# jinlinyi/PerspectiveFields

Measured on NVIDIA H100. Metric: images/sec at 640x480 (Paramnet-360Cities-edina), H100 vs ref CPU, higher is better.
Workload: dtype f32 via 3x bf16 split MMA, fp32 accumulate

## Files before the change

perspectivefields_b200/csrc/gemm_tma.cuh:

```cuda
#pragma once
#include <cuda.h>

#include "tc_ptx.cuh"

namespace pf {

constexpr int MODE_GEMM = 0, MODE_HALO = 1;
constexpr int kTmaThreads = 384;
constexpr int kHaloBytes = 180 * 128;

struct TmaGemmParams {
  int M;
  int B, H, W;
  int Cin;
  int N, K;
  int a_c0, a_gc;
  int c_split, a2_c0;
  int groups;
  int b_row0;
  const float* bias; int bias_mode, bias_gstride;
  int act; const float* gamma;
  const float* res;  int ldr, r_coff, r_gcoff, res_relu;
  const float* res2; int ldr2, r2_coff, r2_gcoff;
  float* C; int ldc, c_coff, c_gcoff;
  __nv_bfloat16* Shi; __nv_bfloat16* Slo; int lds, s_coff, s_gcoff, split_relu;
  const float* pred_w; const float* pred_b; float* pred_out; int pred_nc, pred_mode;
  int phase4;
};

template <int BN, int MODE, int KB, bool PP = false, int NP = 3> struct TmaCfg {
  static_assert(KB == 32 || KB == 64, "KB");
  static_assert(BN % 32 == 0 && BN <= 256, "BN");
  static_assert(!PP || MODE == MODE_GEMM, "the ping-pong schedule is a GEMM-mode schedule");
  static_assert(NP == 1 || NP == 3, "NP");
  static constexpr int kPlanes = NP == 3 ? 2 : 1;
  static constexpr int kTileM = PP ? 64 : 128;
  static constexpr int kBPlane = BN * KB * 2;
  static constexpr int kAPlane = kTileM * KB * 2;
  static constexpr int kStage = (MODE == MODE_GEMM ? kPlanes * kAPlane : 0) + kPlanes * kBPlane;
  static constexpr int kABuf = kPlanes * kHtPlaneBytes;
  static constexpr int kAccPitch = 68;
  static constexpr int kAccStage = 2 * 64 * kAccPitch * 4;
  static constexpr int kBudget = 225 * 1024 - kAccStage - (MODE == MODE_HALO ? 2 * kABuf : 0);
  static constexpr int kStagesRaw = kBudget / kStage;
  static constexpr int kStages = kStagesRaw > 16 ? 16 : kStagesRaw;
  static constexpr int kSmemBytes = (MODE == MODE_HALO ? 2 * kABuf : 0) + kStages * kStage + kAccStage + 512 + 1024;
  static_assert(kStages >= 2, "ring too shallow");
  static_assert(kSmemBytes <= 227 * 1024, "shared memory per block");
};

__device__ __forceinline__ void mbar_expect_tx(uint32_t bar, uint32_t bytes) {
  asm volatile("mbarrier.arrive.expect_tx.shared::cta.b64 _, [%0], %1;\n" ::"r"(bar), "r"(bytes) : "memory");
}
__device__ __forceinline__ void tma_load_2d(uint32_t dst, const CUtensorMap* map, uint32_t bar, int c0, int c1) {
  asm volatile("cp.async.bulk.tensor.2d.shared::cluster.global.mbarrier::complete_tx::bytes [%0], [%1, {%3, %4}], [%2];\n"
               ::"r"(dst), "l"(reinterpret_cast<uint64_t>(map)), "r"(bar), "r"(c0), "r"(c1) : "memory");
}
__device__ __forceinline__ void tma_load_4d(uint32_t dst, const CUtensorMap* map, uint32_t bar, int c0, int c1, int c2, int c3) {
  asm volatile("cp.async.bulk.tensor.4d.shared::cluster.global.mbarrier::complete_tx::bytes [%0], [%1, {%3, %4, %5, %6}], [%2];\n"
               ::"r"(dst), "l"(reinterpret_cast<uint64_t>(map)), "r"(bar), "r"(c0), "r"(c1), "r"(c2), "r"(c3) : "memory");
}
__device__ __forceinline__ void tma_prefetch_desc(const CUtensorMap* map) {
  asm volatile("prefetch.tensormap [%0];\n" ::"l"(reinterpret_cast<uint64_t>(map)) : "memory");
}

struct TmaMaps {
  CUtensorMap a_hi, a_lo, a2_hi, a2_lo, b_hi, b_lo;
};

template <int BN, int MODE, int KB, bool PP = false, int NP = 3>
__global__ void __launch_bounds__(kTmaThreads, 1) gemm_tma_kernel(const __grid_constant__ TmaMaps maps, const TmaGemmParams p, int tiles_x, int tiles_y) {
  using Cfg = TmaCfg<BN, MODE, KB, PP, NP>;
  constexpr bool kLo = NP == 3;
  constexpr int NS = Cfg::kStages;
  constexpr int SPC = 9 * (64 / KB);
  constexpr int kConsumerWarps = PP ? 4 : 8;
  extern __shared__ unsigned char smem_dyn[];
  const uint32_t raw = smem_u32(smem_dyn);
  const uint32_t sbase = (raw + 1023u) & ~1023u;
  unsigned char* sm = smem_dyn + (sbase - raw);
  const uint32_t a_base = sbase;
  const uint32_t ring = sbase + (MODE == MODE_HALO ? 2 * Cfg::kABuf : 0);
  const uint32_t acc_base = ring + NS * Cfg::kStage;
  const uint32_t bars = acc_base + Cfg::kAccStage;
  auto full_b = [&](int s) { return bars + 8u * s; };
  auto empty_b = [&](int s) { return bars + 8u * (NS + s); };
  auto full_a = [&](int i) { return bars + 8u * (2 * NS + i); };
  auto empty_a = [&](int i) { return bars + 8u * (2 * NS + 2 + i); };
  auto order_b = [&](int w) { return bars + 8u * (2 * NS + 4 + w); };

  const int tid = threadIdx.x, lane = tid & 31, warp = tid >> 5;
  const int n_tiles = cdiv(p.N, BN);
  const int m_tiles = MODE == MODE_GEMM ? cdiv(p.M, Cfg::kTileM) : p.B * tiles_x * tiles_y;
  const int total_tiles = m_tiles * n_tiles * p.groups;
  const int nchunks = MODE == MODE_HALO ? p.Cin / 64 : 0;
  const int nk = MODE == MODE_GEMM ? p.K / KB : nchunks * SPC;
  const bool b_resident = MODE == MODE_HALO && nchunks == 1 && SPC <= NS;

  if (tid == 0) {
    tma_prefetch_desc(&maps.a_hi); tma_prefetch_desc(&maps.b_hi);
    if (kLo) { tma_prefetch_desc(&maps.a_lo); tma_prefetch_desc(&maps.b_lo); }
    for (int s = 0; s < NS; ++s) { mbar_init(full_b(s), 1); mbar_init(empty_b(s), kConsumerWarps); }
    for (int i = 0; i < 2; ++i) { mbar_init(full_a(i), 1); mbar_init(empty_a(i), kConsumerWarps); mbar_init(order_b(i), 4); }
    fence_mbar_init();
  }
  __syncthreads();
  pdl_wait();
  pdl_launch();

  auto decode = [&](int tile, int& mt, int& g, int& n0) {
    n0 = (tile % n_tiles) * BN;
    tile /= n_tiles;
    g = tile % p.groups;
    mt = tile / p.groups;
  };

  if (warp < 4) {
    asm volatile("setmaxnreg.dec.sync.aligned.u32 40;\n");
    if (warp == 0 && lane == 0) {
      int it = 0;
      for (int tile = blockIdx.x; tile < total_tiles; tile += gridDim.x) {
        int mt, g, n0;
        decode(tile, mt, g, n0);
        const int brow = p.b_row0 + g * p.N + n0;
        if (b_resident && it > 0) break;
        for (int kc = 0; kc < nk; ++kc, ++it) {
          const int s = it % NS;
          mbar_wait(empty_b(s), ((it / NS) & 1) ^ 1);
          mbar_expect_tx(full_b(s), Cfg::kStage);
          const uint32_t st = ring + s * Cfg::kStage;
          int kcol;
          if (MODE == MODE_GEMM) {
            kcol = kc * KB;
            tma_load_2d(st, &maps.a_hi, full_b(s), p.a_c0 + g * p.a_gc + kcol, mt * Cfg::kTileM);
            if (kLo) tma_load_2d(st + Cfg::kAPlane, &maps.a_lo, full_b(s), p.a_c0 + g * p.a_gc + kcol, mt * Cfg::kTileM);
          } else {
            const int c = kc / SPC, u = kc - c * SPC;
            kcol = KB == 32 ? (u >> 1) * p.Cin + c * 64 + (u & 1) * 32 : u * p.Cin + c * 64;
          }
          const uint32_t bdst = st + (MODE == MODE_GEMM ? Cfg::kPlanes * Cfg::kAPlane : 0);
          tma_load_2d(bdst, &maps.b_hi, full_b(s), kcol, brow);
          if (kLo) tma_load_2d(bdst + Cfg::kBPlane, &maps.b_lo, full_b(s), kcol, brow);
        }
      }
    } else if (MODE == MODE_HALO && warp == 1 && lane == 0) {
      int ita = 0;
      for (int tile = blockIdx.x; tile < total_tiles; tile += gridDim.x) {
        int mt, g, n0;
        decode(tile, mt, g, n0);
        const int tx = mt % tiles_x, ty = (mt / tiles_x) % tiles_y, bimg = mt / (tiles_x * tiles_y);
        for (int c = 0; c < nchunks; ++c, ++ita) {
          const int buf = ita & 1;
          mbar_wait(empty_a(buf), ((ita >> 1) & 1) ^ 1);
          mbar_expect_tx(full_a(buf), Cfg::kPlanes * kHaloBytes);
          const uint32_t dst = a_base + buf * Cfg::kABuf;
          const int ci = c * 64;
          if (p.c_split > 0 && ci >= p.c_split) {
            tma_load_4d(dst, &maps.a2_hi, full_a(buf), p.a2_c0 + ci - p.c_split, tx * kHtTileW - 1, ty * kHtTileH - 1, bimg);
            if (kLo) tma_load_4d(dst + kHtPlaneBytes, &maps.a2_lo, full_a(buf), p.a2_c0 + ci - p.c_split, tx * kHtTileW - 1, ty * kHtTileH - 1, bimg);
          } else {
            tma_load_4d(dst, &maps.a_hi, full_a(buf), p.a_c0 + g * p.a_gc + ci, tx * kHtTileW - 1, ty * kHtTileH - 1, bimg);
            if (kLo) tma_load_4d(dst + kHtPlaneBytes, &maps.a_lo, full_a(buf), p.a_c0 + g * p.a_gc + ci, tx * kHtTileW - 1, ty * kHtTileH - 1, bimg);
          }
        }
      }
    }
    return;
  }

  asm volatile("setmaxnreg.inc.sync.aligned.u32 232;\n");
  const int wg = (warp >> 2) - 1;
  const int wt = tid & 127;
  float* stage = reinterpret_cast<float*>(sm + (acc_base - sbase)) + wg * 64 * Cfg::kAccPitch;
  const int erow = wt & 63, eh = wt >> 6;
  const int r = PP ? erow : wg * 64 + erow;
  constexpr int kTileStep = PP ? 2 : 1;
  float acc[BN / 2];
  int it = 0, ita = 0;
  for (int tl = PP ? wg : 0, tile = blockIdx.x + tl * gridDim.x; tile < total_tiles; tile += kTileStep * gridDim.x, tl += kTileStep) {
    int mt, g, n0;
    decode(tile, mt, g, n0);
    if (PP) {
      it = tl * nk;
      if (tl > 0) mbar_wait(order_b(wg ^ 1), ((tl - 1) >> 1) & 1);
    }
    int prev_s = -1, prev_buf = -1;
    fence_regs(acc);
    for (int kc = 0; kc < nk; ++kc, ++it) {
      const int s = it % NS;
      uint32_t a_hi, a_lo;
      bool chunk_end = false;
      int buf = 0;
      if (MODE == MODE_HALO) {
        const int c = kc / SPC, u = kc - c * SPC;
        const int tap = KB == 32 ? (u >> 1) : u, ky = tap / 3, kx = tap - ky * 3;
        buf = ita & 1;
        if (u == 0) mbar_wait(full_a(buf), (ita >> 1) & 1);
        a_hi = a_base + buf * Cfg::kABuf + ((ky + 8 * wg) * kHtHaloW + kx) * 128 + (KB == 32 ? (u & 1) * 64 : 0);
        a_lo = a_hi + kHtPlaneBytes;
        chunk_end = u == SPC - 1;
      } else {
        a_hi = ring + s * Cfg::kStage + (PP ? 0 : wg * 64 * KB * 2);
        a_lo = a_hi + Cfg::kAPlane;
      }
      const int sb = b_resident ? kc : s;
      if (!b_resident || tl == 0) mbar_wait(full_b(sb), b_resident ? 0 : ((it / NS) & 1));
      const uint32_t b_hi = ring + sb * Cfg::kStage + (MODE == MODE_GEMM ? Cfg::kPlanes * Cfg::kAPlane : 0);
      const uint64_t dah = MODE == MODE_HALO ? ht_a_desc(a_hi) : wgmma_tile_desc<KB>(a_hi);
      const uint64_t dbh = wgmma_tile_desc<KB>(b_hi);
      wgmma_fence();
      if (kLo) {
        const uint64_t dal = MODE == MODE_HALO ? ht_a_desc(a_lo) : wgmma_tile_desc<KB>(a_lo);
        const uint64_t dbl = wgmma_tile_desc<KB>(b_hi + Cfg::kBPlane);
#pragma unroll
        for (int kk = 0; kk < KB / 16; ++kk) {
          const uint32_t first = (kc | kk) ? 1u : 0u;
          wgmma_bf16<BN>(acc, dal + 2 * kk, dbh + 2 * kk, first);
          wgmma_bf16<BN>(acc, dah + 2 * kk, dbl + 2 * kk, 1u);
          wgmma_bf16<BN>(acc, dah + 2 * kk, dbh + 2 * kk, 1u);
        }
      } else {
#pragma unroll
        for (int kk = 0; kk < KB / 16; ++kk) wgmma_bf16<BN>(acc, dah + 2 * kk, dbh + 2 * kk, (kc | kk) ? 1u : 0u);
      }
      wgmma_commit();
      wgmma_wait<1>();
      if (lane == 0 && prev_s >= 0) {
        if (!b_resident) mbar_arrive(empty_b(prev_s));
        if (MODE == MODE_HALO && prev_buf >= 0) mbar_arrive(empty_a(prev_buf));
      }
      prev_s = s;
      prev_buf = chunk_end ? buf : -1;
      if (MODE == MODE_HALO && chunk_end) ++ita;
    }
    if (PP && lane == 0) mbar_arrive(order_b(wg));
    wgmma_wait<0>();
    fence_regs(acc);
    if (lane == 0 && prev_s >= 0) {
      if (!b_resident) mbar_arrive(empty_b(prev_s));
      if (MODE == MODE_HALO && prev_buf >= 0) mbar_arrive(empty_a(prev_buf));
    }

    long long m;
    bool valid;
    int cls_off = 0;
    int bimg = 0, oy = 0, ox = 0;
    if (MODE == MODE_GEMM) {
      m = (long long)mt * Cfg::kTileM + r;
      valid = m < p.M;
    } else {
      const int tx = mt % tiles_x, ty = (mt / tiles_x) % tiles_y;
      bimg = mt / (tiles_x * tiles_y);
      oy = ty * kHtTileH + (r >> 3); ox = tx * kHtTileW + (r & 7);
      valid = oy < p.H && ox < p.W;
      m = ((long long)bimg * p.H + oy) * p.W + ox;
      if (p.bias_mode == 2) {
        const int ry = oy == 0 ? 0 : (oy == p.H - 1 ? 2 : 1);
        const int rx = ox == 0 ? 0 : (ox == p.W - 1 ? 2 : 1);
        cls_off = (ry * 3 + rx) * p.N;
      }
    }
    const float* __restrict__ bias = p.bias ? p.bias + (long long)g * p.bias_gstride : nullptr;
    const int frow = (wt >> 5) * 16 + (lane >> 2), fcol = 2 * (lane & 3);
#pragma unroll
    for (int rd = 0; rd < (BN + 63) / 64; ++rd) {
      named_bar_sync(1 + wg, 128);
#pragma unroll
      for (int jb = 0; jb < 8; ++jb) {
        const int cb = rd * 8 + jb;
        if (cb < BN / 8) {
          float* d0 = stage + frow * Cfg::kAccPitch + jb * 8 + fcol;
          *reinterpret_cast<float2*>(d0) = make_float2(acc[4 * cb], acc[4 * cb + 1]);
          *reinterpret_cast<float2*>(d0 + 8 * Cfg::kAccPitch) = make_float2(acc[4 * cb + 2], acc[4 * cb + 3]);
        }
      }
      named_bar_sync(1 + wg, 128);
      const int ch = 2 * rd + eh;
      const bool ph4 = MODE == MODE_HALO && BN == 128 && p.phase4;
      const bool staged_split = p.Shi && !ph4;
      float o[32];
      if (ch < BN / 32) {
        const int nb = n0 + ch * 32;
        const long long mo = ph4 ? ((long long)bimg * 2 * p.H + 2 * oy + (ch >> 1)) * (2 * p.W) + 2 * ox + (ch & 1) : m;
        const int nbo = ph4 ? 0 : nb;
        const bool chunk_ok = nb < p.N;
        const float* srow = stage + erow * Cfg::kAccPitch + eh * 32;
#pragma unroll
        for (int j = 0; j < 32; j += 4) {
          const float4 t = *reinterpret_cast<const float4*>(srow + j);
          o[j] = t.x; o[j + 1] = t.y; o[j + 2] = t.z; o[j + 3] = t.w;
        }
        if (valid && chunk_ok) {
          if (p.bias_mode) {
#pragma unroll
            for (int j = 0; j < 32; j += 4) {
              const float4 bv = __ldg(reinterpret_cast<const float4*>(bias + cls_off + nb + j));
              o[j] += bv.x; o[j + 1] += bv.y; o[j + 2] += bv.z; o[j + 3] += bv.w;
            }
          }
          if (p.act == 1) {
#pragma unroll
            for (int j = 0; j < 32; ++j) o[j] = fmaxf(o[j], 0.f);
          } else if (p.act == 2) {
#pragma unroll
            for (int j = 0; j < 32; ++j) o[j] = gelu_erf(o[j]);
          }
          if (p.gamma) {
#pragma unroll
            for (int j = 0; j < 32; j += 4) {
              const float4 gv = __ldg(reinterpret_cast<const float4*>(p.gamma + nb + j));
              o[j] *= gv.x; o[j + 1] *= gv.y; o[j + 2] *= gv.z; o[j + 3] *= gv.w;
            }
          }
          if (p.res) {
            const float* rp = p.res + m * p.ldr + p.r_coff + g * p.r_gcoff + nb;
#pragma unroll
            for (int j = 0; j < 32; j += 4) {
              float4 rv = *reinterpret_cast<const float4*>(rp + j);
              if (p.res_relu) { rv.x = fmaxf(rv.x, 0.f); rv.y = fmaxf(rv.y, 0.f); rv.z = fmaxf(rv.z, 0.f); rv.w = fmaxf(rv.w, 0.f); }
              o[j] += rv.x; o[j + 1] += rv.y; o[j + 2] += rv.z; o[j + 3] += rv.w;
            }
          }
          if (p.res2) {
            const float* rp = p.res2 + m * p.ldr2 + p.r2_coff + g * p.r2_gcoff + nb;
#pragma unroll
            for (int j = 0; j < 32; j += 4) {
              const float4 rv = *reinterpret_cast<const float4*>(rp + j);
              o[j] += rv.x; o[j + 1] += rv.y; o[j + 2] += rv.z; o[j + 3] += rv.w;
            }
          }
          if (MODE == MODE_HALO && (BN == 32 || BN == 128) && p.pred_w) {
            float v0 = __ldg(p.pred_b), v1 = p.pred_nc > 1 ? __ldg(p.pred_b + 1) : 0.f;
#pragma unroll
            for (int j = 0; j < 32; j += 4) {
              const float4 w0 = __ldg(reinterpret_cast<const float4*>(p.pred_w + j));
              v0 = fmaf(o[j], w0.x, v0); v0 = fmaf(o[j + 1], w0.y, v0); v0 = fmaf(o[j + 2], w0.z, v0); v0 = fmaf(o[j + 3], w0.w, v0);
              if (p.pred_nc > 1) {
                const float4 w1 = __ldg(reinterpret_cast<const float4*>(p.pred_w + 32 + j));
                v1 = fmaf(o[j], w1.x, v1); v1 = fmaf(o[j + 1], w1.y, v1); v1 = fmaf(o[j + 2], w1.z, v1); v1 = fmaf(o[j + 3], w1.w, v1);
              }
            }
            const long long HWl = (long long)p.H * p.W * (ph4 ? 4 : 1);
            const long long bi = mo / HWl, pix = mo - bi * HWl;
            float* po = p.pred_out + bi * p.pred_nc * HWl + pix;
            if (p.pred_mode == 1) {
              const float nrm = fmaxf(sqrtf(v0 * v0 + v1 * v1), 1e-12f);
              po[0] = v0 / nrm; po[HWl] = v1 / nrm;
            } else {
              po[0] = fminf(fmaxf(v0, -1.f), 1.f);
            }
          }
        }
        if (chunk_ok && (p.C || (p.Shi && !staged_split))) {
          const bool odd = lane & 1;
          const bool valid_p = __shfl_xor_sync(0xffffffffu, (int)valid, 1) != 0;
          const long long mo_p = mo + (odd ? -1 : 1) * (ph4 ? 2 : 1);
          const long long moA = odd ? mo_p : mo, moB = odd ? mo : mo_p;
          const bool vA = odd ? valid_p : valid, vB = odd ? valid : valid_p;
          if (p.C) {
            float* cA = p.C + moA * p.ldc + p.c_coff + g * p.c_gcoff + nbo + (odd ? 4 : 0);
            float* cB = p.C + moB * p.ldc + p.c_coff + g * p.c_gcoff + nbo + (odd ? 4 : 0);
#pragma unroll
            for (int t = 0; t < 4; ++t) {
              float k[4], rr[4];
#pragma unroll
              for (int e = 0; e < 4; ++e) {
                k[e] = odd ? o[8 * t + 4 + e] : o[8 * t + e];
                rr[e] = __shfl_xor_sync(0xffffffffu, odd ? o[8 * t + e] : o[8 * t + 4 + e], 1);
              }
              if (vA) *reinterpret_cast<float4*>(cA + 8 * t) = odd ? make_float4(rr[0], rr[1], rr[2], rr[3]) : make_float4(k[0], k[1], k[2], k[3]);
              if (vB) *reinterpret_cast<float4*>(cB + 8 * t) = odd ? make_float4(k[0], k[1], k[2], k[3]) : make_float4(rr[0], rr[1], rr[2], rr[3]);
            }
          }
          if (p.Shi && !staged_split) {
            const long long sA = moA * p.lds + p.s_coff + g * p.s_gcoff + nbo + (odd ? 8 : 0);
            const long long sB = moB * p.lds + p.s_coff + g * p.s_gcoff + nbo + (odd ? 8 : 0);
#pragma unroll
            for (int t = 0; t < 2; ++t) {
              float k[8], rr[8];
#pragma unroll
              for (int e = 0; e < 8; ++e) {
                const float mine = odd ? o[16 * t + 8 + e] : o[16 * t + e], give = odd ? o[16 * t + e] : o[16 * t + 8 + e];
                k[e] = p.split_relu ? fmaxf(mine, 0.f) : mine;
                rr[e] = __shfl_xor_sync(0xffffffffu, p.split_relu ? fmaxf(give, 0.f) : give, 1);
              }
              uint4 kh, kl, rh, rl;
              split_bf16x2(k[0], k[1], kh.x, kl.x); split_bf16x2(k[2], k[3], kh.y, kl.y);
              split_bf16x2(k[4], k[5], kh.z, kl.z); split_bf16x2(k[6], k[7], kh.w, kl.w);
              split_bf16x2(rr[0], rr[1], rh.x, rl.x); split_bf16x2(rr[2], rr[3], rh.y, rl.y);
              split_bf16x2(rr[4], rr[5], rh.z, rl.z); split_bf16x2(rr[6], rr[7], rh.w, rl.w);
              if (vA) {
                *reinterpret_cast<uint4*>(p.Shi + sA + 16 * t) = odd ? rh : kh;
                *reinterpret_cast<uint4*>(p.Slo + sA + 16 * t) = odd ? rl : kl;
              }
              if (vB) {
                *reinterpret_cast<uint4*>(p.Shi + sB + 16 * t) = odd ? kh : rh;
                *reinterpret_cast<uint4*>(p.Slo + sB + 16 * t) = odd ? kl : rl;
              }
            }
          }
        }
      }
      if (staged_split) {
        named_bar_sync(1 + wg, 128);
        unsigned char* sS = reinterpret_cast<unsigned char*>(stage);
        if (ch < BN / 32) {
#pragma unroll
          for (int t = 0; t < 4; ++t) {
            uint4 h, l;
            float k[8];
#pragma unroll
            for (int e = 0; e < 8; ++e) k[e] = p.split_relu ? fmaxf(o[8 * t + e], 0.f) : o[8 * t + e];
            split_bf16x2(k[0], k[1], h.x, l.x); split_bf16x2(k[2], k[3], h.y, l.y);
            split_bf16x2(k[4], k[5], h.z, l.z); split_bf16x2(k[6], k[7], h.w, l.w);
            const int off = erow * 128 + (((eh * 4 + t) ^ (erow & 7)) << 4);
            *reinterpret_cast<uint4*>(sS + off) = h;
            *reinterpret_cast<uint4*>(sS + 64 * 128 + off) = l;
          }
        }
        named_bar_sync(1 + wg, 128);
#pragma unroll
        for (int i = wt; i < 2 * 64 * 8; i += 128) {
          const int lo_plane = i >> 9, rr = (i >> 3) & 63, pc = i & 7;
          const int col = rd * 64 + pc * 8;
          if (col >= BN || n0 + col >= p.N) continue;
          long long mr;
          bool vr;
          if (MODE == MODE_GEMM) {
            mr = (long long)mt * Cfg::kTileM + (PP ? 0 : wg * 64) + rr;
            vr = mr < p.M;
          } else {
            const int rt = wg * 64 + rr, tx = mt % tiles_x, ty = (mt / tiles_x) % tiles_y;
            const int py = ty * kHtTileH + (rt >> 3), px = tx * kHtTileW + (rt & 7);
            vr = py < p.H && px < p.W;
            mr = ((long long)bimg * p.H + py) * p.W + px;
          }
          if (!vr) continue;
          const uint4 v = *reinterpret_cast<const uint4*>(sS + lo_plane * 64 * 128 + rr * 128 + ((pc ^ (rr & 7)) << 4));
          *reinterpret_cast<uint4*>((lo_plane ? p.Slo : p.Shi) + mr * p.lds + p.s_coff + g * p.s_gcoff + n0 + col) = v;
        }
      }
    }
  }
}

}
```

Measured before the change: 786.9.

## Stage residual loads and fp32 output stores through shared memory for coalescing

Residual and second-residual tensors are now loaded cooperatively into shared memory with row-contiguous float4 accesses, then read back per thread, rather than each thread loading its own 32-float row segment. The non-phase4 fp32 C output is likewise written back to the staging buffer and stored with coalesced row-major float4 writes instead of shuffle-paired scattered stores. Row index computation is factored into a helper lambda. This targets uncoalesced global traffic in the epilogue, at the cost of extra named barriers and shared-memory round trips per chunk.

```diff
diff --git a/perspectivefields_b200/csrc/gemm_tma.cuh b/perspectivefields_b200/csrc/gemm_tma.cuh
--- a/perspectivefields_b200/csrc/gemm_tma.cuh
+++ b/perspectivefields_b200/csrc/gemm_tma.cuh
@@ -244,14 +244,15 @@
     long long m;
     bool valid;
     int cls_off = 0;
-    int bimg = 0, oy = 0, ox = 0;
+    int bimg = 0, oy = 0, ox = 0, oy0 = 0, ox0 = 0;
     if (MODE == MODE_GEMM) {
       m = (long long)mt * Cfg::kTileM + r;
       valid = m < p.M;
     } else {
       const int tx = mt % tiles_x, ty = (mt / tiles_x) % tiles_y;
       bimg = mt / (tiles_x * tiles_y);
-      oy = ty * kHtTileH + (r >> 3); ox = tx * kHtTileW + (r & 7);
+      oy0 = ty * kHtTileH; ox0 = tx * kHtTileW;
+      oy = oy0 + (r >> 3); ox = ox0 + (r & 7);
       valid = oy < p.H && ox < p.W;
       m = ((long long)bimg * p.H + oy) * p.W + ox;
       if (p.bias_mode == 2) {
@@ -261,6 +262,15 @@
       }
     }
     const float* __restrict__ bias = p.bias ? p.bias + (long long)g * p.bias_gstride : nullptr;
+    auto stage_row = [&](int rr, long long& mr) -> bool {
+      if (MODE == MODE_GEMM) {
+        mr = (long long)mt * Cfg::kTileM + (PP ? 0 : wg * 64) + rr;
+        return mr < p.M;
+      }
+      const int rt = wg * 64 + rr, py = oy0 + (rt >> 3), px = ox0 + (rt & 7);
+      mr = ((long long)bimg * p.H + py) * p.W + px;
+      return py < p.H && px < p.W;
+    };
     const int frow = (wt >> 5) * 16 + (lane >> 2), fcol = 2 * (lane & 3);
 #pragma unroll
     for (int rd = 0; rd < (BN + 63) / 64; ++rd) {
@@ -276,135 +286,174 @@
       }
       named_bar_sync(1 + wg, 128);
       const int ch = 2 * rd + eh;
+      const bool own = ch < BN / 32;
       const bool ph4 = MODE == MODE_HALO && BN == 128 && p.phase4;
       const bool staged_split = p.Shi && !ph4;
+      const int nb = n0 + ch * 32;
+      const bool chunk_ok = own && nb < p.N;
+      const bool live = valid && chunk_ok;
+      const float* srow = stage + erow * Cfg::kAccPitch + eh * 32;
       float o[32];
-      if (ch < BN / 32) {
-        const int nb = n0 + ch * 32;
-        const long long mo = ph4 ? ((long long)bimg * 2 * p.H + 2 * oy + (ch >> 1)) * (2 * p.W) + 2 * ox + (ch & 1) : m;
-        const int nbo = ph4 ? 0 : nb;
-        const bool chunk_ok = nb < p.N;
-        const float* srow = stage + erow * Cfg::kAccPitch + eh * 32;
+      if (own) {
 #pragma unroll
         for (int j = 0; j < 32; j += 4) {
           const float4 t = *reinterpret_cast<const float4*>(srow + j);
           o[j] = t.x; o[j + 1] = t.y; o[j + 2] = t.z; o[j + 3] = t.w;
         }
-        if (valid && chunk_ok) {
-          if (p.bias_mode) {
-#pragma unroll
-            for (int j = 0; j < 32; j += 4) {
-              const float4 bv = __ldg(reinterpret_cast<const float4*>(bias + cls_off + nb + j));
-              o[j] += bv.x; o[j + 1] += bv.y; o[j + 2] += bv.z; o[j + 3] += bv.w;
+      }
+      if (live) {
+        if (p.bias_mode) {
+#pragma unroll
+          for (int j = 0; j < 32; j += 4) {
+            const float4 bv = __ldg(reinterpret_cast<const float4*>(bias + cls_off + nb + j));
+            o[j] += bv.x; o[j + 1] += bv.y; o[j + 2] += bv.z; o[j + 3] += bv.w;
+          }
+        }
+        if (p.act == 1) {
+#pragma unroll
+          for (int j = 0; j < 32; ++j) o[j] = fmaxf(o[j], 0.f);
+        } else if (p.act == 2) {
+#pragma unroll
+          for (int j = 0; j < 32; ++j) o[j] = gelu_erf(o[j]);
+        }
+        if (p.gamma) {
+#pragma unroll
+          for (int j = 0; j < 32; j += 4) {
+            const float4 gv = __ldg(reinterpret_cast<const float4*>(p.gamma + nb + j));
+            o[j] *= gv.x; o[j + 1] *= gv.y; o[j + 2] *= gv.z; o[j + 3] *= gv.w;
+          }
+        }
+      }
+      auto stage_in = [&](const float* src, int ld, int coff) {
+        named_bar_sync(1 + wg, 128);
+        float4 v[8];
+#pragma unroll
+        for (int t = 0; t < 8; ++t) {
+          const int i = wt + 128 * t, col = rd * 64 + (i & 15) * 4;
+          long long mr;
+          v[t] = make_float4(0.f, 0.f, 0.f, 0.f);
+          if (col < BN && n0 + col < p.N && stage_row(i >> 4, mr)) v[t] = *reinterpret_cast<const float4*>(src + mr * ld + coff + n0 + col);
+        }
+#pragma unroll
+        for (int t = 0; t < 8; ++t) {
+          const int i = wt + 128 * t;
+          *reinterpret_cast<float4*>(stage + (i >> 4) * Cfg::kAccPitch + (i & 15) * 4) = v[t];
+        }
+        named_bar_sync(1 + wg, 128);
+      };
+      if (p.res) {
+        stage_in(p.res, p.ldr, p.r_coff + g * p.r_gcoff);
+        if (live) {
+#pragma unroll
+          for (int j = 0; j < 32; j += 4) {
+            float4 rv = *reinterpret_cast<const float4*>(srow + j);
+            if (p.res_relu) { rv.x = fmaxf(rv.x, 0.f); rv.y = fmaxf(rv.y, 0.f); rv.z = fmaxf(rv.z, 0.f); rv.w = fmaxf(rv.w, 0.f); }
+            o[j] += rv.x; o[j + 1] += rv.y; o[j + 2] += rv.z; o[j + 3] += rv.w;
+          }
+        }
+      }
+      if (p.res2) {
+        stage_in(p.res2, p.ldr2, p.r2_coff + g * p.r2_gcoff);
+        if (live) {
+#pragma unroll
+          for (int j = 0; j < 32; j += 4) {
+            const float4 rv = *reinterpret_cast<const float4*>(srow + j);
+            o[j] += rv.x; o[j + 1] += rv.y; o[j + 2] += rv.z; o[j + 3] += rv.w;
+          }
+        }
+      }
+      const long long mo = ph4 ? ((long long)bimg * 2 * p.H + 2 * oy + (ch >> 1)) * (2 * p.W) + 2 * ox + (ch & 1) : m;
+      if (MODE == MODE_HALO && (BN == 32 || BN == 128) && p.pred_w && live) {
+        float v0 = __ldg(p.pred_b), v1 = p.pred_nc > 1 ? __ldg(p.pred_b + 1) : 0.f;
+#pragma unroll
+        for (int j = 0; j < 32; j += 4) {
+          const float4 w0 = __ldg(reinterpret_cast<const float4*>(p.pred_w + j));
+          v0 = fmaf(o[j], w0.x, v0); v0 = fmaf(o[j + 1], w0.y, v0); v0 = fmaf(o[j + 2], w0.z, v0); v0 = fmaf(o[j + 3], w0.w, v0);
+          if (p.pred_nc > 1) {
+            const float4 w1 = __ldg(reinterpret_cast<const float4*>(p.pred_w + 32 + j));
+            v1 = fmaf(o[j], w1.x, v1); v1 = fmaf(o[j + 1], w1.y, v1); v1 = fmaf(o[j + 2], w1.z, v1); v1 = fmaf(o[j + 3], w1.w, v1);
+          }
+        }
+        const long long HWl = (long long)p.H * p.W * (ph4 ? 4 : 1);
+        const long long bi = mo / HWl, pix = mo - bi * HWl;
+        float* po = p.pred_out + bi * p.pred_nc * HWl + pix;
+        if (p.pred_mode == 1) {
+          const float nrm = fmaxf(sqrtf(v0 * v0 + v1 * v1), 1e-12f);
+          po[0] = v0 / nrm; po[HWl] = v1 / nrm;
+        } else {
+          po[0] = fminf(fmaxf(v0, -1.f), 1.f);
+        }
+      }
+      if (ph4 && chunk_ok && (p.C || p.Shi)) {
+        const bool odd = lane & 1;
+        const bool valid_p = __shfl_xor_sync(0xffffffffu, (int)valid, 1) != 0;
+        const long long mo_p = mo + (odd ? -2 : 2);
+        const long long moA = odd ? mo_p : mo, moB = odd ? mo : mo_p;
+        const bool vA = odd ? valid_p : valid, vB = odd ? valid : valid_p;
+        if (p.C) {
+          float* cA = p.C + moA * p.ldc + p.c_coff + g * p.c_gcoff + (odd ? 4 : 0);
+          float* cB = p.C + moB * p.ldc + p.c_coff + g * p.c_gcoff + (odd ? 4 : 0);
+#pragma unroll
+          for (int t = 0; t < 4; ++t) {
+            float k[4], rr[4];
+#pragma unroll
+            for (int e = 0; e < 4; ++e) {
+              k[e] = odd ? o[8 * t + 4 + e] : o[8 * t + e];
+              rr[e] = __shfl_xor_sync(0xffffffffu, odd ? o[8 * t + e] : o[8 * t + 4 + e], 1);
             }
-          }
-          if (p.act == 1) {
-#pragma unroll
-            for (int j = 0; j < 32; ++j) o[j] = fmaxf(o[j], 0.f);
-          } else if (p.act == 2) {
-#pragma unroll
-            for (int j = 0; j < 32; ++j) o[j] = gelu_erf(o[j]);
-          }
-          if (p.gamma) {
-#pragma unroll
-            for (int j = 0; j < 32; j += 4) {
-              const float4 gv = __ldg(reinterpret_cast<const float4*>(p.gamma + nb + j));
-              o[j] *= gv.x; o[j + 1] *= gv.y; o[j + 2] *= gv.z; o[j + 3] *= gv.w;
+            if (vA) *reinterpret_cast<float4*>(cA + 8 * t) = odd ? make_float4(rr[0], rr[1], rr[2], rr[3]) : make_float4(k[0], k[1], k[2], k[3]);
+            if (vB) *reinterpret_cast<float4*>(cB + 8 * t) = odd ? make_float4(k[0], k[1], k[2], k[3]) : make_float4(rr[0], rr[1], rr[2], rr[3]);
+          }
+        }
+        if (p.Shi) {
+          const long long sA = moA * p.lds + p.s_coff + g * p.s_gcoff + (odd ? 8 : 0);
+          const long long sB = moB * p.lds + p.s_coff + g * p.s_gcoff + (odd ? 8 : 0);
+#pragma unroll
+          for (int t = 0; t < 2; ++t) {
+            float k[8], rr[8];
+#pragma unroll
+            for (int e = 0; e < 8; ++e) {
+              const float mine = odd ? o[16 * t + 8 + e] : o[16 * t + e], give = odd ? o[16 * t + e] : o[16 * t + 8 + e];
+              k[e] = p.split_relu ? fmaxf(mine, 0.f) : mine;
+              rr[e] = __shfl_xor_sync(0xffffffffu, p.split_relu ? fmaxf(give, 0.f) : give, 1);
             }
-          }
-          if (p.res) {
-            const float* rp = p.res + m * p.ldr + p.r_coff + g * p.r_gcoff + nb;
-#pragma unroll
-            for (int j = 0; j < 32; j += 4) {
-              float4 rv = *reinterpret_cast<const float4*>(rp + j);
-              if (p.res_relu) { rv.x = fmaxf(rv.x, 0.f); rv.y = fmaxf(rv.y, 0.f); rv.z = fmaxf(rv.z, 0.f); rv.w = fmaxf(rv.w, 0.f); }
-              o[j] += rv.x; o[j + 1] += rv.y; o[j + 2] += rv.z; o[j + 3] += rv.w;
+            uint4 kh, kl, rh, rl;
+            split_bf16x2(k[0], k[1], kh.x, kl.x); split_bf16x2(k[2], k[3], kh.y, kl.y);
+            split_bf16x2(k[4], k[5], kh.z, kl.z); split_bf16x2(k[6], k[7], kh.w, kl.w);
+            split_bf16x2(rr[0], rr[1], rh.x, rl.x); split_bf16x2(rr[2], rr[3], rh.y, rl.y);
+            split_bf16x2(rr[4], rr[5], rh.z, rl.z); split_bf16x2(rr[6], rr[7], rh.w, rl.w);
+            if (vA) {
+              *reinterpret_cast<uint4*>(p.Shi + sA + 16 * t) = odd ? rh : kh;
+              *reinterpret_cast<uint4*>(p.Slo + sA + 16 * t) = odd ? rl : kl;
             }
-          }
-          if (p.res2) {
-            const float* rp = p.res2 + m * p.ldr2 + p.r2_coff + g * p.r2_gcoff + nb;
-#pragma unroll
-            for (int j = 0; j < 32; j += 4) {
-              const float4 rv = *reinterpret_cast<const float4*>(rp + j);
-              o[j] += rv.x; o[j + 1] += rv.y; o[j + 2] += rv.z; o[j + 3] += rv.w;
+            if (vB) {
+              *reinterpret_cast<uint4*>(p.Shi + sB + 16 * t) = odd ? kh : rh;
+              *reinterpret_cast<uint4*>(p.Slo + sB + 16 * t) = odd ? kl : rl;
             }
           }
-          if (MODE == MODE_HALO && (BN == 32 || BN == 128) && p.pred_w) {
-            float v0 = __ldg(p.pred_b), v1 = p.pred_nc > 1 ? __ldg(p.pred_b + 1) : 0.f;
-#pragma unroll
-            for (int j = 0; j < 32; j += 4) {
-              const float4 w0 = __ldg(reinterpret_cast<const float4*>(p.pred_w + j));
-              v0 = fmaf(o[j], w0.x, v0); v0 = fmaf(o[j + 1], w0.y, v0); v0 = fmaf(o[j + 2], w0.z, v0); v0 = fmaf(o[j + 3], w0.w, v0);
-              if (p.pred_nc > 1) {
-                const float4 w1 = __ldg(reinterpret_cast<const float4*>(p.pred_w + 32 + j));
-                v1 = fmaf(o[j], w1.x, v1); v1 = fmaf(o[j + 1], w1.y, v1); v1 = fmaf(o[j + 2], w1.z, v1); v1 = fmaf(o[j + 3], w1.w, v1);
-              }
-            }
-            const long long HWl = (long long)p.H * p.W * (ph4 ? 4 : 1);
-            const long long bi = mo / HWl, pix = mo - bi * HWl;
-            float* po = p.pred_out + bi * p.pred_nc * HWl + pix;
-            if (p.pred_mode == 1) {
-              const float nrm = fmaxf(sqrtf(v0 * v0 + v1 * v1), 1e-12f);
-              po[0] = v0 / nrm; po[HWl] = v1 / nrm;
-            } else {
-              po[0] = fminf(fmaxf(v0, -1.f), 1.f);
-            }
-          }
-        }
-        if (chunk_ok && (p.C || (p.Shi && !staged_split))) {
-          const bool odd = lane & 1;
-          const bool valid_p = __shfl_xor_sync(0xffffffffu, (int)valid, 1) != 0;
-          const long long mo_p = mo + (odd ? -1 : 1) * (ph4 ? 2 : 1);
-          const long long moA = odd ? mo_p : mo, moB = odd ? mo : mo_p;
-          const bool vA = odd ? valid_p : valid, vB = odd ? valid : valid_p;
-          if (p.C) {
-            float* cA = p.C + moA * p.ldc + p.c_coff + g * p.c_gcoff + nbo + (odd ? 4 : 0);
-            float* cB = p.C + moB * p.ldc + p.c_coff + g * p.c_gcoff + nbo + (odd ? 4 : 0);
-#pragma unroll
-            for (int t = 0; t < 4; ++t) {
-              float k[4], rr[4];
-#pragma unroll
-              for (int e = 0; e < 4; ++e) {
-                k[e] = odd ? o[8 * t + 4 + e] : o[8 * t + e];
-                rr[e] = __shfl_xor_sync(0xffffffffu, odd ? o[8 * t + e] : o[8 * t + 4 + e], 1);
-              }
-              if (vA) *reinterpret_cast<float4*>(cA + 8 * t) = odd ? make_float4(rr[0], rr[1], rr[2], rr[3]) : make_float4(k[0], k[1], k[2], k[3]);
-              if (vB) *reinterpret_cast<float4*>(cB + 8 * t) = odd ? make_float4(k[0], k[1], k[2], k[3]) : make_float4(rr[0], rr[1], rr[2], rr[3]);
-            }
-          }
-          if (p.Shi && !staged_split) {
-            const long long sA = moA * p.lds + p.s_coff + g * p.s_gcoff + nbo + (odd ? 8 : 0);
-            const long long sB = moB * p.lds + p.s_coff + g * p.s_gcoff + nbo + (odd ? 8 : 0);
-#pragma unroll
-            for (int t = 0; t < 2; ++t) {
-              float k[8], rr[8];
-#pragma unroll
-              for (int e = 0; e < 8; ++e) {
-                const float mine = odd ? o[16 * t + 8 + e] : o[16 * t + e], give = odd ? o[16 * t + e] : o[16 * t + 8 + e];
-                k[e] = p.split_relu ? fmaxf(mine, 0.f) : mine;
-                rr[e] = __shfl_xor_sync(0xffffffffu, p.split_relu ? fmaxf(give, 0.f) : give, 1);
-              }
-              uint4 kh, kl, rh, rl;
-              split_bf16x2(k[0], k[1], kh.x, kl.x); split_bf16x2(k[2], k[3], kh.y, kl.y);
-              split_bf16x2(k[4], k[5], kh.z, kl.z); split_bf16x2(k[6], k[7], kh.w, kl.w);
-              split_bf16x2(rr[0], rr[1], rh.x, rl.x); split_bf16x2(rr[2], rr[3], rh.y, rl.y);
-              split_bf16x2(rr[4], rr[5], rh.z, rl.z); split_bf16x2(rr[6], rr[7], rh.w, rl.w);
-              if (vA) {
-                *reinterpret_cast<uint4*>(p.Shi + sA + 16 * t) = odd ? rh : kh;
-                *reinterpret_cast<uint4*>(p.Slo + sA + 16 * t) = odd ? rl : kl;
-              }
-              if (vB) {
-                *reinterpret_cast<uint4*>(p.Shi + sB + 16 * t) = odd ? kh : rh;
-                *reinterpret_cast<uint4*>(p.Slo + sB + 16 * t) = odd ? kl : rl;
-              }
-            }
-          }
+        }
+      }
+      if (p.C && !ph4) {
+        named_bar_sync(1 + wg, 128);
+        if (own) {
+          float* drow = stage + erow * Cfg::kAccPitch + eh * 32;
+#pragma unroll
+          for (int j = 0; j < 32; j += 4) *reinterpret_cast<float4*>(drow + j) = make_float4(o[j], o[j + 1], o[j + 2], o[j + 3]);
+        }
+        named_bar_sync(1 + wg, 128);
+        float* cbase = p.C + p.c_coff + g * p.c_gcoff + n0;
+#pragma unroll
+        for (int t = 0; t < 8; ++t) {
+          const int i = wt + 128 * t, col = rd * 64 + (i & 15) * 4;
+          long long mr;
+          if (col < BN && n0 + col < p.N && stage_row(i >> 4, mr))
+            *reinterpret_cast<float4*>(cbase + mr * p.ldc + col) = *reinterpret_cast<const float4*>(stage + (i >> 4) * Cfg::kAccPitch + (i & 15) * 4);
         }
       }
       if (staged_split) {
         named_bar_sync(1 + wg, 128);
         unsigned char* sS = reinterpret_cast<unsigned char*>(stage);
-        if (ch < BN / 32) {
+        if (own) {
 #pragma unroll
           for (int t = 0; t < 4; ++t) {
             uint4 h, l;
@@ -423,19 +472,8 @@
         for (int i = wt; i < 2 * 64 * 8; i += 128) {
           const int lo_plane = i >> 9, rr = (i >> 3) & 63, pc = i & 7;
           const int col = rd * 64 + pc * 8;
-          if (col >= BN || n0 + col >= p.N) continue;
           long long mr;
-          bool vr;
-          if (MODE == MODE_GEMM) {
-            mr = (long long)mt * Cfg::kTileM + (PP ? 0 : wg * 64) + rr;
-            vr = mr < p.M;
-          } else {
-            const int rt = wg * 64 + rr, tx = mt % tiles_x, ty = (mt / tiles_x) % tiles_y;
-            const int py = ty * kHtTileH + (rt >> 3), px = tx * kHtTileW + (rt & 7);
-            vr = py < p.H && px < p.W;
-            mr = ((long long)bimg * p.H + py) * p.W + px;
-          }
-          if (!vr) continue;
+          if (col >= BN || n0 + col >= p.N || !stage_row(rr, mr)) continue;
           const uint4 v = *reinterpret_cast<const uint4*>(sS + lo_plane * 64 * 128 + rr * 128 + ((pc ^ (rr & 7)) << 4));
           *reinterpret_cast<uint4*>((lo_plane ? p.Slo : p.Shi) + mr * p.lds + p.s_coff + g * p.s_gcoff + n0 + col) = v;
         }
```

Result: faster. 812.6 (median of 6 runs) (+3.3%).
